# truemeat001/Simple-Raytracing-Render

Measured on AMD Instinct MI355X. Metric: Msamples/s (rays x bounces) + HBM GB/s vs roofline, Cornell+teapot 1024spp, higher is better.
Workload: dtype f32

## Files before the change

include/srr_capi.h:

```cpp
#ifndef SRR_CAPI_H
#define SRR_CAPI_H

#include <stddef.h>
#include <stdint.h>

#ifdef __cplusplus
extern "C" {
#endif

#define SRR_OK 0
#define SRR_EINVAL (-22)
#define SRR_ENOMEM (-12)
#define SRR_ENODEV (-19)
#define SRR_ENOTSUP (-95)
#define SRR_EIO (-5)

typedef struct srr_scene srr_scene;
typedef struct srr_renderer srr_renderer;

const char* srr_last_error(void);
const char* srr_version(void);

srr_scene* srr_scene_create(void);
void srr_scene_destroy(srr_scene* s);
int srr_scene_from_text(const char* text, srr_scene** out);
int srr_scene_text_handle(const srr_scene* s, int text_id);
int srr_scene_set_lcg(srr_scene* s, uint64_t state);
#define SRR_DIGEST_PARTS 21
int srr_scene_digest(const srr_scene* s, uint64_t* out, uint64_t* parts);
uint64_t srr_scene_get_lcg(const srr_scene* s);
double srr_scene_drand48(srr_scene* s);

int srr_constant_texture(srr_scene* s, float r, float g, float b);
int srr_image_texture(srr_scene* s, const unsigned char* rgb, int nx, int ny);
int srr_image_texture_file(srr_scene* s, const char* path);
int srr_image_texture_gen(srr_scene* s, int nx, int ny, uint32_t seed, int kind);
int srr_checker_texture(srr_scene* s, int even_tex, int odd_tex);
int srr_noise_texture(srr_scene* s, float scale);

int srr_lambertian(srr_scene* s, int albedo_tex);
int srr_orennayar(srr_scene* s, int albedo_tex, float sigma_deg);
int srr_beckmann(srr_scene* s, int albedo_tex, float roughx, float roughy);
int srr_metal(srr_scene* s, float r, float g, float b, float fuzz);
int srr_dielectric(srr_scene* s, float ref_idx);
int srr_diffuse_light(srr_scene* s, int emit_tex);
int srr_isotropic(srr_scene* s, int albedo_tex);

int srr_sphere(srr_scene* s, const float center[3], float radius, int mat);
int srr_moving_sphere(srr_scene* s, const float c0[3], const float c1[3], float t0, float t1, float radius,
                      int mat);
int srr_xy_rect(srr_scene* s, float x0, float x1, float y0, float y1, float k, int mat);
int srr_xz_rect(srr_scene* s, float x0, float x1, float z0, float z1, float k, int mat);
int srr_yz_rect(srr_scene* s, float y0, float y1, float z0, float z1, float k, int mat);
int srr_box(srr_scene* s, const float p0[3], const float p1[3], int mat);
int srr_triangle(srr_scene* s, const float p[9], int mat, const float* uv9, const float* n9);
int srr_flip_normals(srr_scene* s, int child);
int srr_translate(srr_scene* s, int child, const float offset[3]);
int srr_rotate_y(srr_scene* s, int child, float angle_deg);
int srr_rotate_x(srr_scene* s, int child, float angle_deg);
int srr_constant_medium(srr_scene* s, int boundary, float density, int tex);
int srr_hitable_list(srr_scene* s, const int* children, int n);
int srr_bvh_node(srr_scene* s, const int* children, int n, float time0, float time1);
int srr_teapot(srr_scene* s, float scale, int divs, int mat, int* first_handle);

int srr_model(srr_scene* s, const char* path, int flip_uvs, int flip_winding, int mat, const float scale[3],
              int* first_handle);
int srr_mesh_file_triangles(const char* path, int flip_uvs, int flip_winding, const float scale[3], float* pos9,
                            float* uv9, float* nrm9, int* flags_out);

int srr_camera(srr_scene* s, const float lookfrom[3], const float lookat[3], const float vup[3], float vfov,
               float aspect, float aperture, float focus_dist, float t0, float t1);
int srr_scene_set_world(srr_scene* s, int obj);
int srr_scene_set_lights(srr_scene* s, int list_obj);

typedef struct srr_params {
  int nx, ny;
  int spp;
  int max_depth;
  int tile;
  int shard_index;
  int shard_count;
  int batch_paths;
// ... 112 lines not shown
```

simple-raytracing-render_amd/csrc/capi.cpp:

```cpp
#include <hip/hip_runtime.h>

#include <algorithm>
#include <chrono>
#include <cstdint>
#include <cstdio>
#include <cstring>
#include <map>
#include <memory>
#include <mutex>
#include <string>
#include <vector>

#include "../../include/srr_capi.h"
#include "denoise.h"
#include "imageio.h"
#include "meshio.h"
#include "../../include/srr/merl.h"
#include "multi.h"
#include "renderer.h"

using namespace srr;

struct srr_scene {
  Scene s;
// ... 53 lines not shown
  std::string err;
  const int rc = flatten(s->s, f, err);
  if (rc < 0) return fail(rc, err);
  uint64_t h = 0xcbf29ce484222325ULL;
  int part = 0;
  auto mix = [](uint64_t& x, const void* p, size_t n) {
    const unsigned char* b = (const unsigned char*)p;
    for (size_t i = 0; i < n; ++i) x = (x ^ b[i]) * 0x100000001b3ULL;
  };
  auto blob = [&](const void* p, size_t n) {
    mix(h, &n, sizeof n);
    mix(h, p, n);
    if (const char* dd = getenv("SRR_DIGEST_DUMP")) {
      FILE* df = fopen((std::string(dd) + "." + std::to_string(part)).c_str(), "wb");
      if (df) { fwrite(p, 1, n, df); fclose(df); }
    }
    if (parts) {
      uint64_t x = 0xcbf29ce484222325ULL;
      mix(x, p, n);
      parts[part] = x;
    }
    ++part;
  };
  auto vec = [&blob](const auto& v) { blob(v.data(), v.size() * sizeof(v[0])); };
  vec(f.objs);
  blob(&f.n_world, sizeof f.n_world);
  vec(f.xforms);
  vec(f.spheres);
  vec(f.rects);
  vec(f.stris);
  vec(f.meshes);
  vec(f.nodes);
  vec(f.node4);
  vec(f.tri_pos);
  vec(f.tri_shade);
  vec(f.media);
  {
    std::vector<uint8_t> b;
    auto put = [&b](const void* p, size_t n) { b.insert(b.end(), (const uint8_t*)p, (const uint8_t*)p + n); };
    put(f.obvhs.data(), f.obvhs.size() * sizeof(DObvh));
    put(f.sgroups.data(), f.sgroups.size() * sizeof(DSGroup));
    put(f.sg_items.data(), f.sg_items.size() * sizeof(DSGItem));
    vec(b);
  }
  vec(f.obvh_children);
  vec(f.mats);
  vec(f.texs);
  vec(f.images);
  vec(f.perlin_ranvec);
  vec(f.perlin_perm);
  vec(f.lights);
  blob(&f.cam, sizeof f.cam);
  *out = h;
  return 0;
}

int srr_scene_set_lcg(srr_scene* s, uint64_t state) {
  if (!s) return fail(SRR_EINVAL, "null scene");
  s->s.lcg = state & 0xFFFFFFFFFFFFULL;
  return 0;
}
uint64_t srr_scene_get_lcg(const srr_scene* s) { return s ? s->s.lcg : 0; }
double srr_scene_drand48(srr_scene* s) { return s ? s->s.drand48() : 0.0; }

#define SCN(s) \
  if (!(s)) return fail(SRR_EINVAL, "null scene");
#define TEXOK(s, t) \
  if (!(s)->s.valid_tex(t)) return fail(SRR_EINVAL, "bad texture handle " + std::to_string(t));
#define MATOK(s, m) \
  if (!(s)->s.valid_mat(m)) return fail(SRR_EINVAL, "bad material handle " + std::to_string(m));
#define OBJOK(s, o) \
  if (!(s)->s.valid_obj(o)) return fail(SRR_EINVAL, "bad hitable handle " + std::to_string(o));

int srr_constant_texture(srr_scene* s, float r, float g, float b) {
  SCN(s);
  HTex t;
  t.kind = TEX_CONST;
  t.c[0] = r; t.c[1] = g; t.c[2] = b;
  return s->s.add_tex(std::move(t));
}
int srr_image_texture(srr_scene* s, const unsigned char* rgb, int nx, int ny) {
  SCN(s);
  if (!rgb || nx <= 0 || ny <= 0) return fail(SRR_EINVAL, "bad image");
  HTex t;
  t.kind = TEX_IMAGE;
  t.nx = nx;
  t.ny = ny;
  t.px.assign(rgb, rgb + (size_t)nx * ny * 3);
  return s->s.add_tex(std::move(t));
}
int srr_image_texture_file(srr_scene* s, const char* path) {
  SCN(s);
  if (!path) return fail(SRR_EINVAL, "null path");
  srr::Image im;
  std::string err;
  if (srr::load_image(path, 0, im, err) < 0) return fail(SRR_EIO, err);
  if (im.n < 3) return fail(SRR_EINVAL, std::string(path) + ": image_texture needs 3 or 4 channels");
  HTex t;
  t.kind = TEX_IMAGE;
  t.nx = im.w;
  t.ny = im.h;
  t.px.assign(im.px.begin(), im.px.begin() + (size_t)im.w * im.h * 3);
  return s->s.add_tex(std::move(t));
}
int srr_image_texture_gen(srr_scene* s, int nx, int ny, uint32_t seed, int kind) {
  SCN(s);
// ... 1088 lines not shown
```

simple-raytracing-render_amd/csrc/device_scene.h:

```cpp
#pragma once
#include <cstdint>

namespace srr {

enum ObjKind : int32_t {
  OBJ_SPHERE = 0,
  OBJ_MSPHERE = 1,
  OBJ_RECT = 2,
  OBJ_TRI = 3,
  OBJ_MESH = 4,
  OBJ_MEDIUM = 5,
  OBJ_OBVH = 6,
  OBJ_SGROUP = 7,
};

enum XformKind : int32_t { XF_FLIP = 0, XF_TRANSLATE = 1, XF_ROTY = 2, XF_ROTX = 3 };

struct DXform {
  int32_t kind;
  float a, b, c;
};


constexpr int32_t kXfFlipBit = 1 << 30;
constexpr int32_t kXfCountMask = 0xFFFF;

struct DObj {
  int32_t kind;
  int32_t xf_begin, xf_count;
  int32_t idx;
};

struct DSphere {
  float c0[3], c1[3];
  float t0, t1, r;
  int32_t mat;
};

struct DRect {
  int32_t kax, a0, a1, mat;
  float lo0, hi0, lo1, hi1, k;
  float pad[3];
};

struct TriShade {
  float n[9];
  float uv[6];
  int32_t mat;
};

constexpr int kNode4qWords = 16;

struct DMesh {
  int32_t node_off;
  int32_t tri_off;
  int32_t n_nodes, n_tris;
  int32_t node4_off;
  int32_t n_node4;
};

struct DObvh {
  int32_t node_off, n_nodes;
  int32_t child_off, n_children;
};

struct DObvhChild {
  int32_t obj_begin, obj_count;
};

constexpr int kSGroupMinRun = 8;

struct DSGroup {
  int32_t node_off, n_nodes;
  int32_t item_off, n_items;
};

struct DSGItem {
  DSphere s;
  int32_t pos;
  int32_t moving;
  int32_t obj;
  int32_t pad;
};

struct DMedium {
  int32_t bnd_begin, bnd_count;
  float density;
  int32_t phase_mat;
};

enum MatKind : int32_t {
  MAT_LAMBERTIAN = 0,
  MAT_ORENNAYAR = 1,
  MAT_BECKMANN = 2,
  MAT_METAL = 3,
  MAT_DIELECTRIC = 4,
// ... 40 lines not shown
```

simple-raytracing-render_amd/csrc/kernels.h:

```cpp
#pragma once
#include <hip/hip_runtime.h>

#include <cstdint>

#include "device_scene.h"

namespace srr {

struct SceneView {
  const DObj* objs;
  int n_world;
  int has_media;
  const DXform* xforms;
  const DSphere* spheres;
  const DRect* rects;
  const DStandaloneTri* stris;
  const DMesh* meshes;
  const float4* nodes;
  const float4* node4;
  int node4_lds;
  int node4_total;
  const float4* node4q;
  int node4_lds_q;
  int use_q;
  int quad_trace;
  int quad_max;
  int mesh_obj;
  const float4* tri_pos;
  const float4* tri_edge;
  const TriShade* tri_shade;
  const DMedium* media;
  const DObvh* obvhs;
  const DObvhChild* obvh_children;
  const DSGroup* sgroups;
  const DSGItem* sg_items;
  const DMat* mats;
  const DTex* texs;
  const uint8_t* images;
  const float* perlin_ranvec;
  const int32_t* perlin_perm;
  const DLight* lights;
  int n_lights;
  float light_weight;
  const DCamera* cam;
  const uint4* world_blob;
  int world_words;
  int world_off[10];
};

struct PathState {
  float4* ray_o;
  float4* ray_d;
  uint64_t* lcg;
  uint64_t* pcg;
  int32_t* depth;
  uint64_t* spec;
  int4* hit_w;
  float4* hit_p;
  float4* hit_n;
  float4* rec_a;
  float* sample;
  float* raw;
  uint8_t* rays;
};

struct BatchInfo {
  int32_t* active;
  int32_t* count;
  int act0;
  int slot0;
  const int32_t* pixels;
  const double* sobol;
  int p0;
  int n_paths;
  int s0, spp_batch;
  int s_base;
  int nx, ny;
  uint64_t base_seed;
};

struct UDiv31 {
  uint32_t m, p;
};
inline UDiv31 make_udiv31(uint32_t d) {
  uint32_t l = 0;
  while ((1ull << l) < d) ++l;
  const uint32_t p = 31 + l;
  return UDiv31{(uint32_t)(((1ull << p) + d - 1) / d), p};
}

struct PathWork {
  const int32_t* pixels;
  const double* sobol;
  int npix, spp_w;
  int s_base;
  int nx, ny;
  UDiv31 div_spp, div_nx;
  uint64_t base_seed;
  int64_t n_paths;
  int max_depth;
// ... 207 lines not shown
```

simple-raytracing-render_amd/csrc/kernels.hip:

```cpp
#include <hip/hip_runtime.h>

#include <cfloat>
#include <algorithm>
#include <cstdint>
#include <cstdlib>
#include <cstring>

#include "device_scene.h"
#include "devmath.h"
#include "kernels.h"
#include "../../include/srr/merl.h"

namespace srr {
namespace dev {

SRR_D V3 sphere_center(const DSphere& s, float tm, bool moving) {
  V3 c0 = v3(s.c0[0], s.c0[1], s.c0[2]);
  if (!moving) return c0;
  V3 c1 = v3(s.c1[0], s.c1[1], s.c1[2]);
  return c0 + ((tm - s.t0) / (s.t1 - s.t0)) * (c1 - c0);
}

SRR_D bool sphere_hit(const DSphere& s, bool moving, const Ray& r, float tmin, float tmax, float& t) {
  V3 oc = r.o - sphere_center(s, r.tm, moving);
// ... 598 lines not shown
    atomicAdd(cx.ctr + 1, (unsigned long long)ntri);
    if (overflow) atomicAdd(cx.ctr + 2, 1ull);
    const int steps = (int)(nbox / 4);
    atomicAdd(cx.ctr + 3 + min(steps, 63), 1ull);
    int wmax = steps;
    for (int o = 32; o > 0; o >>= 1) wmax = max(wmax, __shfl_xor(wmax, o));
    if ((int)__lane_id() == __ffsll((unsigned long long)__ballot(1)) - 1) atomicAdd(cx.ctr + 67 + min(wmax, 63), 1ull);
  }
  if (TIMING) {
    sp2 += __builtin_amdgcn_s_memtime() - ts;
    {
      int lm = (int)nbox;
      for (int o = 32; o > 0; o >>= 1) lm = max(lm, __shfl_xor(lm, o));
      const int src = __ffsll((unsigned long long)__ballot((int)nbox == lm)) - 1;
      cx.step_parts[0] += (uint64_t)__shfl((unsigned long long)sp0, src);
      cx.step_parts[1] += (uint64_t)__shfl((unsigned long long)sp1, src);
      cx.step_parts[2] += (uint64_t)__shfl((unsigned long long)sp2, src);
      cx.leaf_cycles += (uint64_t)__shfl((unsigned long long)slf, src);
      cx.leaf_passes += __shfl(spass, src);
    }
    int st = (int)(nbox / 4), sum = st, walk = st > 0;
    for (int o = 32; o > 0; o >>= 1) {
      st = max(st, __shfl_xor(st, o));
      sum += __shfl_xor(sum, o);
      walk += __shfl_xor(walk, o);
    }
    cx.mesh_steps += st;
    cx.mesh_lane_steps += sum;
    cx.mesh_walkers += walk;
    cx.mesh_cycles += __builtin_amdgcn_s_memtime() - tm_enter;
  }
  if (cx.ovf && cx.gst) {
    const uint64_t dm = __ballot(deep && !suspended);
    if (dm && (int)__lane_id() == __ffsll((unsigned long long)dm) - 1) atomicAdd(cx.ovf + (kCtrDeepTraversals - kCtrStackOverflows), (unsigned long long)__popcll(dm));
  }
#ifdef SRR_SLOW_RAYS
  cx.last_steps += (int)(nbox / 4) | (overflow ? 1 << 30 : 0) | (deep ? 1 << 29 : 0);
#endif
  if (SUSP && suspended) return false;
  if (overflow) {
    if (cx.ovf) atomicAdd(cx.ovf, 1ull);
    return mesh_hit<false>(S, m, r, tmin, tmax, is_medium, out, cx.ctr);
  }
  out.t = best_t;
  out.tri = best_i;
  return found;
}

constexpr int TR_QUAD = 32;
constexpr int TR_Q = 64;
constexpr int TR_BIG = 128;
constexpr int tr_stride(int tr) { return (tr & TR_BIG) ? 1024 : kTraceBlock; }
constexpr int TR_SUSP = 256;

template <int CTRL>
SRR_D int quad_dpp(int x) { return __builtin_amdgcn_update_dpp(x, x, CTRL, 0xF, 0xF, false); }
template <int CTRL>
SRR_D float quad_dpp(float x) { return __int_as_float(quad_dpp<CTRL>(__float_as_int(x))); }
constexpr int kQuadXor1 = 0xB1, kQuadXor2 = 0x4E;
template <int K>
constexpr int kQuadBcast = K * 0x55;

SRR_D void quad_best(bool& f, float& t, int& i) {
#define SRR_QSTEP(CTRL)                                                      \
  {                                                                          \
    const bool of = quad_dpp<CTRL>((int)f) != 0;                             \
    const float ot = quad_dpp<CTRL>(t);                                      \
    const int oi = quad_dpp<CTRL>(i);                                        \
    if (of && (!f || wins(ot, oi, t, i))) { f = true; t = ot; i = oi; }       \
  }
  SRR_QSTEP(kQuadXor1) SRR_QSTEP(kQuadXor2)
#undef SRR_QSTEP
}

template <bool PRUNE, int STRIDE = kTraceBlock>
SRR_D bool mesh_hit4_quad(const SceneView& S, const DMesh& m, const Ray& r, float tmin, float tmax, bool is_medium,
                          MeshHit& out, const TraceCtx& cx) {
  if (const uint64_t nanm = __ballot(!(tmax == tmax))) {
    bool f = false;
    float bt = 0;
    int bi = -1;
    mesh_scan_nan(S, m, r, is_medium, nanm, f, bt, bi);
    if (!(tmax == tmax)) {
#ifdef SRR_SLOW_RAYS
      cx.last_steps |= 1 << 28;
#endif
      out.t = bt;
      out.tri = bi;
      return f;
    }
  }
  const V3 inv = v3(1.0f / r.d.x, 1.0f / r.d.y, 1.0f / r.d.z);
  const bool want = slab(S.nodes[2 * m.node_off], S.nodes[2 * m.node_off + 1], r.o, inv, tmin, tmax);
  if (__ballot(1) != ~0ull) {
    if (!want) return false;
    return mesh_hit4<PRUNE, false, false, STRIDE>(S, m, r, tmin, tmax, is_medium, out, cx);
  }
  const int lane = __lane_id(), q = lane >> 2, c = lane & 3;
  const float len = length(r.d);
  const V3 dir = r.d / len;
  const float to_param = kPruneSlack / len;
  const int gslot = cx.slot - c;
  bool found_me = false, redo_me = false;
  float t_me = 0;
  int i_me = -1;
  uint64_t W = __ballot(want);
// ... 409 lines not shown
  float lo = -FLT_MAX;
#pragma unroll 1
  for (int pass = 0; pass < 2; ++pass) {
    float th;
    if (!list_hit<TR>(S, md.bnd_begin, md.bnd_count, r, lo, FLT_MAX, th, cx)) return false;
    tb[pass] = th;
    lo = (float)((double)th + 0.0001);
  }
  float t1 = tb[0], t2 = tb[1];
  if (t1 < tmin) t1 = tmin;
  if (t2 > tmax) t2 = tmax;
  if (t1 >= t2) return false;
  if (t1 < 0) t1 = 0;
  float len = length(r.d);
  float inside = (t2 - t1) * len;
  float hit_distance = -(1 / md.density) * gm64::log(drand(rng));
  if (hit_distance < inside) {
    t = t1 + hit_distance / len;
    return true;
  }
  return false;
}

struct WorldHit {
  int obj;
  int prim;
  float t;
};

template <bool MEDIA, int TR>
SRR_D void world_objs(const SceneView& S, const Ray& r, Rng& rng, const TraceCtx& cx, int k0, int k1, WorldHit& w,
                      float& closest) {
  const float tmin = 0.001f;
  for (int k = k0; k < k1; ++k) {
    const DObj ob = uni(wload<TR>(S.objs, k));
    Ray lr = chain_in<TR, true>(S, ob, r);
    ObjHit h;
    bool hit;
    if (MEDIA && ob.kind == OBJ_MEDIUM) {
      hit = medium_hit<TR>(S, uni(wload<TR>(S.media, ob.idx)), lr, tmin, closest, rng, h.t, cx);
      h.prim = -1;
    } else {
      hit = basic_hit<TR, true>(S, ob, lr, tmin, closest, false, h, cx);
    }
    if (hit) {
      closest = h.t;
      w.obj = k;
      w.prim = h.prim;
      w.t = h.t;
    }
  }
}

template <bool MEDIA, int TR>
SRR_D WorldHit world_hit(const SceneView& S, const Ray& r, Rng& rng, const TraceCtx& cx) {
  WorldHit w{-1, -1, 0};
  float closest = FLT_MAX;
  const float tmin = 0.001f;
  constexpr bool SUSP = (TR & TR_SUSP) != 0;
  const bool skip = MEDIA || S.mesh_obj < 0;
  int k_res = -1;
  if constexpr (SUSP) {
    if (skip && cx.resume) {
      const float4 v = *walk_save(cx, 2);
      k_res = __float_as_int(v.x);
      closest = v.y;
      w.obj = __float_as_int(v.z);
      w.prim = __float_as_int(v.w);
      w.t = closest;
    }
  }
  for (int k = 0; k < S.n_world; ++k) {
    const DObj ob = uni(wload<TR>(S.objs, k));
    if constexpr (SUSP) {
      if (skip && (cx.susp || k < k_res)) continue;
      cx.obj_k = k;
    }
    Ray lr = chain_in<TR, true>(S, ob, r);
    ObjHit h;
    bool hit;
    if (MEDIA && ob.kind == OBJ_MEDIUM) {
      hit = medium_hit<TR>(S, uni(wload<TR>(S.media, ob.idx)), lr, tmin, closest, rng, h.t, cx);
      h.prim = -1;
    } else {
      hit = basic_hit<TR, true>(S, ob, lr, tmin, closest, false, h, cx);
    }
    if (SUSP && skip && cx.susp) {
      *walk_save(cx, 2) = make_float4(__int_as_float(k), closest, __int_as_float(w.obj), __int_as_float(w.prim));
      continue;
    }
    if (hit) {
      closest = h.t;
      w.obj = k;
      w.prim = h.prim;
      w.t = h.t;
    }
  }
  return w;
}

struct HitRec {
  V3 p, n;
  float u, v;
  int mat;
};

template <int KAX>
SRR_D void rect_rec(const DRect& q, const Ray& r, HitRec& h) {
  constexpr int A0 = KAX == 0 ? 1 : 0, A1 = KAX == 2 ? 1 : 2;
  const float tt = (q.k - r.o[KAX]) / r.d[KAX];
  const float x = r.o[A0] + tt * r.d[A0];
  const float y = r.o[A1] + tt * r.d[A1];
  h.u = (x - q.lo0) / (q.hi0 - q.lo0);
  h.v = (y - q.lo1) / (q.hi1 - q.lo1);
  h.n = v3(0.f);
  h.n.set(KAX, 1.f);
}

SRR_D void sphere_uv(V3 p, float& u, float& v) {
  float phi = ratan2(p.z, p.x);
  float theta = rasin(p.y);
  u = 1 - (phi + kPi) / (2 * kPi);
  v = (theta + kPi / 2) / kPi;
}

// ... 1436 lines not shown
      e[12] = __int_as_float(wh.prim);
      e[13] = wh.t;
      e[14] = __int_as_float(slot);
      e[15] = __int_as_float((int)(t_w0 & 0x7fffffff));
    }
  }
}
#endif

constexpr int kTpWords = 8, kTfWords = kCtrBeckAttemptsMax - kCtrTicksBeck + 1, kTzWords = 2, kTptWords = 3;
constexpr int kTpPhases = kCtrTicksFold - kCtrTicksRefill + 1;
template <int Q>
constexpr int tp_at() {
  constexpr int at = Q >= kCtrTicksRefill && Q <= kCtrTicksFold ? Q - kCtrTicksRefill
                     : Q == kCtrTicksRecord ? kTpPhases : Q == kCtrTicksMixture ? kTpPhases + 1
                     : Q == kCtrMixtureRounds ? kTpPhases + 2 : -1;
  static_assert(at >= 0 && at < kTpWords, "not a word of tp");
  return at;
}
template <int Q>
constexpr int tf_at() {
  static_assert(Q >= kCtrTicksBeck && Q <= kCtrBeckAttemptsMax, "not a word of tf");
  return Q - kCtrTicksBeck;
}
template <int Q>
constexpr int tz_at() {
  static_assert(Q >= kCtrTicksCamOnly && Q < kCtrTicksCamOnly + kTzWords, "not a word of tz");
  return Q - kCtrTicksCamOnly;
}
template <int Q>
constexpr int tpt_at() {
  static_assert(Q >= kCtrTicksPretrace && Q < kCtrTicksPretrace + kTptWords, "not a word of tpt");
  return Q - kCtrTicksPretrace;
}
constexpr int kThtWords = kCtrTailLanes - kCtrTicksHead + 1;
constexpr int kHeadLiveMin = 32;

template <bool MEDIA, bool ALLFAM, int MINB, bool TIMED = false, bool WL = true, bool QUAD = false, bool CQ = false,
          int BS = kPathsBlock, bool SP = false>
#ifdef SRR_NUM_VGPR
#define SRR_PATHS_VGPR_ATTR __attribute__((amdgpu_num_vgpr(SRR_NUM_VGPR)))
#else
#define SRR_PATHS_VGPR_ATTR
#endif
__global__ void __launch_bounds__(BS, MINB) SRR_PATHS_VGPR_ATTR k_paths(PathsArgs A) {
  static_assert(BS == kPathsBlock || BS == 1024, "block size");
  (void)A;
  uint64_t tp[kTpWords] = {0, 0, 0, 0, 0, 0, 0, 0};
  uint64_t tf[kTfWords] = {0, 0, 0, 0, 0, 0, 0, 0, 0, 0, 0, 0, 0, 0, 0, 0, 0, 0, 0, 0};
  uint64_t tz[kTzWords] = {0, 0};
  uint64_t it = 0;
  uint64_t tpt[kTptWords] = {0, 0, 0};
  constexpr int TR = TR_BVH4_PRUNE | (WL ? TR_WL : 0) | (QUAD ? TR_QUAD : 0) | (CQ ? TR_Q : 0) | (BS == 1024 ? TR_BIG : 0) |
                     ((SP && !QUAD && !CQ) ? TR_SUSP : 0);
  __shared__ uint4 s_world[WL ? kWorldLdsBytes / 16 : 1];
  const auto view = [&]() {
    SceneView S = paths_args()->S;
    if constexpr (WL) {
      const char* b = (const char*)s_world;
      S.objs = (const DObj*)(b + S.world_off[0]);
      S.xforms = (const DXform*)(b + S.world_off[1]);
      S.spheres = (const DSphere*)(b + S.world_off[2]);
      S.rects = (const DRect*)(b + S.world_off[3]);
      S.stris = (const DStandaloneTri*)(b + S.world_off[4]);
      S.meshes = (const DMesh*)(b + S.world_off[5]);
      S.media = (const DMedium*)(b + S.world_off[6]);
      S.mats = (const DMat*)(b + S.world_off[7]);
      S.texs = (const DTex*)(b + S.world_off[8]);
      S.lights = (const DLight*)(b + S.world_off[9]);
    }
    return S;
  };
  const auto work = []() { return PathWork(paths_args()->W); };
  __shared__ int s_node[kStack * BS];
  __shared__ float s_t[kStack * BS];
  constexpr bool RING = !QUAD;
  constexpr bool PT = RING && !MEDIA && !ALLFAM && (BS == 1024 || TIMED);
  constexpr int kRingWords = ring_words(PT);
  constexpr int kNodesLds = paths_lds_nodes(BS, WL, RING, PT);
  static_assert(paths_lds_fits(BS, WL, RING, PT), "k_paths LDS");
  __shared__ float4 s_n4[kNodesLds * 8];
  __shared__ float s_ring[RING ? kRingWords * BS : 1];
  static_assert(sizeof(s_world) + sizeof(s_node) + sizeof(s_t) + sizeof(s_n4) + sizeof(s_ring) ==
                    (size_t)paths_lds_bytes(BS, WL, RING, PT), "k_paths LDS as kernels.h counts it");
  const auto lds_nodes = [](const SceneView& S) { return min(S.node4_total, (CQ ? 2 : 1) * kNodesLds); };
  const lds_ptr<float> ringw = to_lds(s_ring + (RING ? (threadIdx.x & ~63u) : 0));
  uint32_t ring_base = 0;
  const uint32_t n_paths = (uint32_t)paths_args()->W.n_paths;
  const uint64_t t_start = paths_args()->W.wave_times ? __builtin_amdgcn_s_memrealtime() : 0;
  {
    const SceneView S0 = paths_args()->S;
    if constexpr (WL)
      for (int i = threadIdx.x; i < S0.world_words; i += blockDim.x) s_world[i] = S0.world_blob[i];
    const int n_lds_nodes = lds_nodes(S0);
    if (CQ)
      for (int i = threadIdx.x; i < n_lds_nodes * 4; i += blockDim.x) s_n4[i] = S0.node4q[i];
    else
      for (int i = threadIdx.x; i < n_lds_nodes * 8; i += blockDim.x) s_n4[i] = S0.node4[i];
  }
  __syncthreads();
  const int slot = blockIdx.x * blockDim.x + threadIdx.x;
  const auto rec_at = [&](const PathWork& W, int k) -> float4* {
    int s = slot;
    asm volatile("" : "+v"(s));
    return W.rec + ((size_t)k * W.lanes + s);
  };
  int g = -1;
// ... 134 lines not shown
          if (lane_id() == 0) b = (uint32_t)atomicAdd(W.cursor, (unsigned long long)kPoolChunk);
          nb = __builtin_amdgcn_readfirstlane(b);
        }
        idx = rank < avail ? pool + rank : nb + (rank - avail);
        pool = nb + (cnt - avail);
        pool_end = nb + (uint32_t)kPoolChunk;
      }
      if (!RING && need && idx < n_paths) {
        g = (int)idx;
        path_camera_ray(S, W, idx, r, rng);
        depth = 0;
      }
    }
    if (!nxt_armed && pool_end < n_paths) {
      nxt_lane0 = pool_arm(nxt_lane0);
      nxt_armed = true;
    }
    if (__ballot(g >= 0) == 0) break;
    if (TIMED) tf[tf_at<kCtrLanesInPath>()] += __popcll(__ballot(g >= 0));
    if (TIMED) {
      __builtin_amdgcn_s_waitcnt(0);
      const uint64_t t = __builtin_amdgcn_s_memtime();
      tp[tp_at<kCtrTicksRefill>()] += t - tq;
      tq = t;
      ++it;
    }
    }
    const bool head_now = PT && !tail;
    const bool act = g >= 0;
    const Ray tr = r;
    if (act) {
      const SceneView S = view();
      const PathWork W = work();
      TraceCtx cx{nullptr, to_lds(s_node + threadIdx.x), to_lds(s_t + threadIdx.x)};
      cx.lds_nodes = (const __attribute__((address_space(3))) f32x4*)to_lds(s_n4);
      cx.lds_count = lds_nodes(S);
      cx.st_cap = min(W.stack_cap, kStack);
      cx.ovf = W.counters + kCtrStackOverflows;
      cx.gst = W.gstack;
      cx.gst_cap = W.gstack ? W.gstack_cap : 0;
      cx.gst_stride = W.lanes;
      cx.slot = slot;
      if constexpr ((TR & TR_SUSP) != 0) {
        cx.walk_thr = vreg(head_now ? 0 : (int)((__popcll(__ballot(true)) * (uint32_t)paths_args()->W.walk_q) >> 6));
        cx.resume = walking;
        cx.susp = vreg(0);
      }
#ifdef SRR_SLOW_RAYS
      const uint64_t t_w0 = __builtin_amdgcn_s_memrealtime();
      cx.last_steps = 0;
      const Ray r_in = tr;
#endif
      const WorldHit wh =
          world_hit<MEDIA, TIMED ? (TR_BVH4_TIMED | (WL ? TR_WL : 0) | (SP ? TR_SUSP : 0)) : TR>(S, tr, rng, cx);
      w = wh;
      if constexpr ((TR & TR_SUSP) != 0) {
        walking = cx.susp;
        if (walking) {
          w.obj = -1;
          n_events += kSuspended;
        }
      }
#ifdef SRR_SLOW_RAYS
      slow_ray_record(W, g, depth, r_in, t_w0, cx.last_steps, wh, slot);
#endif
      if (TIMED) {
        const uint64_t t = __builtin_amdgcn_s_memtime();
        if (head_now && passes == 0) {
          tpt[tpt_at<kCtrTicksPretrace>()] += t - tq;
          ++tpt[tpt_at<kCtrPretracePasses>()];
        } else {
          if (__ballot(depth != 0) == 0) {
            tz[tz_at<kCtrTicksCamOnly>()] += t - tq;
            ++tz[tz_at<kCtrItsCamOnly>()];
          }
          tp[tp_at<kCtrTicksWorld>()] += t - tq - cx.mesh_cycles;
          tp[tp_at<kCtrTicksMesh>()] += cx.mesh_cycles;
          tf[tf_at<kCtrMeshSteps>()] += cx.mesh_steps;
          tf[tf_at<kCtrMeshLaneSteps>()] += cx.mesh_lane_steps;
          tf[tf_at<kCtrMeshWalkers>()] += cx.mesh_walkers;
          tf[tf_at<kCtrLeafTicks>()] += cx.leaf_cycles;
          tf[tf_at<kCtrLeafPasses>()] += cx.leaf_passes;
          tf[tf_at<kCtrStepFetch>()] += cx.step_parts[0];
          tf[tf_at<kCtrStepSlab>()] += cx.step_parts[1];
          tf[tf_at<kCtrStepOrder>()] += cx.step_parts[2];
        }
        tq = t;
      }
    }
    if (nxt_armed && !nxt_ready) {
      nxt_base = __builtin_amdgcn_readfirstlane(nxt_lane0);
      nxt_ready = true;
    }
    {
    const bool sh = g >= 0 && !(PT && walking);
    if (PT && TIMED) ++tpt[tpt_at<kCtrShadeRounds>()];
    bool done = sh && !walking;
    V3 C = v3(0.f);
    bool diff = false, pend = false;
    int natt = 0;
    uint64_t fam_dt[3] = {0, 0, 0};
    DiffSetup ds{};
    V3 d_atten = v3(0.f), d_n = v3(0.f), d_dir = v3(0.f);
    float d_pdf = 0;
    int d_tries = 0;
    bool d_dead = false;
    if (sh) {
// ... 1254 lines not shown
```

simple-raytracing-render_amd/csrc/renderer.cpp:

```cpp
#include "renderer.h"

#include "multi.h"

#include <algorithm>
#include <chrono>
#include <cstdlib>
#include <cstring>
#include <memory>
#include <thread>
#include <cstdio>

namespace srr {

constexpr int kVisitWords = 3 + 2 * 64;

#define RCHK(x)                                                        \
  do {                                                                 \
    hipError_t e_ = (x);                                               \
    if (e_ != hipSuccess) {                                            \
      err = std::string(#x) + ": " + hipGetErrorString(e_);            \
      return SRR_EIO;                                                  \
    }                                                                  \
  } while (0)

// ... 19 lines not shown
  r->device = device;
  if (const char* e = getenv("SRR_LANES")) r->n_lanes = std::max(1, std::min(kMaxLanes, atoi(e)));
  RCHK(hipSetDevice(device));
  std::vector<void*>& K = r->scene_bufs;
  DObj* objs; DXform* xf; DSphere* sph; DRect* rct; DStandaloneTri* st; DMesh* me; float* nodes; float* n4;
  float* tp; TriShade* ts; DMedium* md; DMat* mt; DTex* tx; uint8_t* im; float* pr; int32_t* pp; DLight* li;
  DCamera* cm;
  DObvh* ob;
  DObvhChild* oc;
  DSGroup* sg;
  DSGItem* sgi;
  std::vector<DCamera> cam{F.cam};
  RCHK(upload(&objs, F.objs, K));
  RCHK(upload(&xf, F.xforms, K));
  RCHK(upload(&sph, F.spheres, K));
  RCHK(upload(&rct, F.rects, K));
  RCHK(upload(&st, F.stris, K));
  RCHK(upload(&me, F.meshes, K));
  RCHK(upload(&nodes, F.nodes, K));
  RCHK(upload(&n4, F.node4, K));
  float* n4q;
  RCHK(upload(&n4q, F.node4q, K));
  RCHK(upload(&tp, F.tri_pos, K));
  float* tedge;
  {
    const size_t nt = F.tri_pos.size() / 16;
    std::vector<float> pr(32 * nt, 0.f);
    for (size_t i = 0; i < nt; ++i)
      for (int j = 0; j < 2; ++j) {
        const float* q = &F.tri_pos[16 * std::min(i + j, nt - 1)];
        float* o = &pr[32 * i + 9 * j];
        for (int c = 0; c < 3; ++c) {
          o[c] = q[c];
          o[3 + c] = q[4 + c] - q[c];
          o[6 + c] = q[8 + c] - q[c];
        }
      }
    RCHK(upload(&tedge, pr, K));
  }
  RCHK(upload(&ts, F.tri_shade, K));
  RCHK(upload(&md, F.media, K));
  RCHK(upload(&ob, F.obvhs, K));
  RCHK(upload(&oc, F.obvh_children, K));
  RCHK(upload(&sg, F.sgroups, K));
  RCHK(upload(&sgi, F.sg_items, K));
  RCHK(upload(&mt, F.mats, K));
  RCHK(upload(&tx, F.texs, K));
  RCHK(upload(&im, F.images, K));
  RCHK(upload(&pr, F.perlin_ranvec, K));
  RCHK(upload(&pp, F.perlin_perm, K));
  RCHK(upload(&li, F.lights, K));
  RCHK(upload(&cm, cam, K));
  std::vector<uint8_t> blob;
  int off[10];
  auto put = [&](int k, const void* data, size_t bytes) {
    off[k] = (int)blob.size();
    blob.insert(blob.end(), (const uint8_t*)data, (const uint8_t*)data + bytes);
    blob.resize((blob.size() + 15) & ~(size_t)15, 0);
  };
  put(0, F.objs.data(), F.objs.size() * sizeof(DObj));
  put(1, F.xforms.data(), F.xforms.size() * sizeof(DXform));
  put(2, F.spheres.data(), F.spheres.size() * sizeof(DSphere));
  put(3, F.rects.data(), F.rects.size() * sizeof(DRect));
  put(4, F.stris.data(), F.stris.size() * sizeof(DStandaloneTri));
  put(5, F.meshes.data(), F.meshes.size() * sizeof(DMesh));
  put(6, F.media.data(), F.media.size() * sizeof(DMedium));
  put(7, F.mats.data(), F.mats.size() * sizeof(DMat));
  put(8, F.texs.data(), F.texs.size() * sizeof(DTex));
  put(9, F.lights.data(), F.lights.size() * sizeof(DLight));
  uint8_t* wb;
  RCHK(upload(&wb, blob, K));
  SceneView& V = r->view;
  V.world_blob = (const uint4*)wb;
  V.world_words = (int)(blob.size() / 16);
  for (int k = 0; k < 10; ++k) V.world_off[k] = off[k];
  V.objs = objs;
  V.n_world = F.n_world;
  V.has_media = F.media.empty() ? 0 : 1;
  V.xforms = xf;
  V.spheres = sph;
  V.rects = rct;
  V.stris = st;
  V.meshes = me;
  V.nodes = (const float4*)nodes;
  V.node4 = (const float4*)n4;
  V.node4_lds = (int)std::min<size_t>(kPathsLdsNodes, F.node4.size() / 32);
  V.node4_total = (int)(F.node4.size() / 32);
  V.node4q = F.node4q_ok && !F.node4q.empty() ? (const float4*)n4q : nullptr;
  V.node4_lds_q = (int)std::min<size_t>(2 * kPathsLdsNodes, F.node4q.size() / kNode4qWords);
  {
    const char* e = getenv("SRR_CBVH");
    V.use_q = V.node4q && e && atoi(e) != 0;
  }
  {
    const char* e = getenv("SRR_QUAD");
    V.quad_trace = e ? (atoi(e) != 0) : false;
    const char* q = getenv("SRR_QUAD_MAX");
    V.quad_max = q ? atoi(q) : 32;
  }
  {
    int n_mesh = 0;
    V.mesh_obj = -1;
    for (int k = 0; k < F.n_world; ++k)
      if (F.objs[k].kind == OBJ_MESH) {
        ++n_mesh;
        V.mesh_obj = k;
      }
    if (n_mesh != 1) V.mesh_obj = -1;
  }
  V.tri_pos = (const float4*)tp;
  V.tri_edge = (const float4*)tedge;
  V.tri_shade = ts;
  V.media = md;
  V.obvhs = ob;
  V.obvh_children = oc;
  V.sgroups = sg;
  V.sg_items = sgi;
  V.mats = mt;
  V.texs = tx;
  V.images = im;
  V.perlin_ranvec = pr;
  V.perlin_perm = pp;
  V.lights = li;
  V.n_lights = (int)F.lights.size();
  V.light_weight = V.n_lights > 0 ? (float)(1.0 / V.n_lights) : 0.f;
  V.cam = cm;
  r->has_meshes = !F.meshes.empty() || !F.obvhs.empty();
  r->diffuse_only = true;
// ... 1185 lines not shown
```

simple-raytracing-render_amd/csrc/scene.cpp:

```cpp
#include "scene.h"

#include <algorithm>
#include <array>
#include <cfloat>
#include <cmath>
#include <cstdio>
#include <cstdlib>
#include <cstring>
#include <fstream>
#include <functional>
#include <iterator>
#include <map>
#include <sstream>

namespace srr {

static const double kPi = 3.14159265358979323846;
static const uint64_t kPostPerlinSeed = 24561125610955ULL;

#include "../../include/srr/teapot_data.inc"

Scene::Scene() : lcg(kPostPerlinSeed) {}

double Scene::drand48() {
// ... 1317 lines not shown
    g.item_off = (int)F.sg_items.size();
    g.n_items = (int)items.size();
    std::vector<float> nodes;
    std::function<void(int, int)> build = [&](int lo, int hi) {
      double mn[3] = {INFINITY, INFINITY, INFINITY}, mx[3] = {-INFINITY, -INFINITY, -INFINITY};
      double cmn[3] = {INFINITY, INFINITY, INFINITY}, cmx[3] = {-INFINITY, -INFINITY, -INFINITY};
      for (int k = lo; k < hi; ++k)
        for (int a = 0; a < 3; ++a) {
          mn[a] = std::min(mn[a], items[k].mn[a]);
          mx[a] = std::max(mx[a], items[k].mx[a]);
          cmn[a] = std::min(cmn[a], items[k].c[a]);
          cmx[a] = std::max(cmx[a], items[k].c[a]);
        }
      const size_t me = nodes.size() / 8;
      nodes.resize(nodes.size() + 8);
      for (int a = 0; a < 3; ++a) {
        float fl = (float)mn[a], fh = (float)mx[a];
        if ((double)fl > mn[a]) fl = std::nextafter(fl, -INFINITY);
        if ((double)fh < mx[a]) fh = std::nextafter(fh, INFINITY);
        nodes[8 * me + a] = fl;
        nodes[8 * me + 4 + a] = fh;
      }
      int32_t leaf = -1;
      if (hi - lo <= 2) {
        leaf = ((int)F.sg_items.size() << 1) | (hi - lo - 1);
        for (int k = lo; k < hi; ++k) F.sg_items.push_back(items[k].it);
      } else {
        int ax = 0;
        for (int a = 1; a < 3; ++a)
          if (cmx[a] - cmn[a] > cmx[ax] - cmn[ax]) ax = a;
        const int mid = (lo + hi) / 2;
        std::nth_element(items.begin() + lo, items.begin() + mid, items.begin() + hi,
                         [ax](const It& x, const It& y) { return x.c[ax] < y.c[ax]; });
        build(lo, mid);
        build(mid, hi);
      }
      const int32_t skip = g.node_off + (int32_t)(nodes.size() / 8);
      std::memcpy(&nodes[8 * me + 3], &skip, 4);
      std::memcpy(&nodes[8 * me + 7], &leaf, 4);
    };
    build(0, (int)items.size());
    g.n_nodes = (int)(nodes.size() / 8);
    F.nodes.insert(F.nodes.end(), nodes.begin(), nodes.end());
    F.sgroups.push_back(g);
    DObj d{};
    d.kind = OBJ_SGROUP;
    d.idx = (int)F.sgroups.size() - 1;
    out.push_back(d);
    i = j;
  }
  return out;
}

int flatten(const Scene& S, Flat& F, std::string& err) {
  F = Flat();
  if (S.world < 0 || S.lights < 0 || !S.has_camera) {
    err = "scene needs world, lights and a camera";
    return -22;
  }
  if (S.obj[S.lights].kind != H_LIST) {
    err = "lights must be a hitable_list (Raytracing_n.cpp:75 casts it)";
    return -22;
  }
  for (const HMat& m : S.mat) {
    DMat d{};
    d.kind = m.kind;
    d.tex = m.tex;
    std::memcpy(d.p, m.p, 16);
    F.mats.push_back(d);
  }
  for (const HTex& t : S.tex) {
    DTex d{};
    d.kind = t.kind;
    std::memcpy(d.c, t.c, 12);
    d.nx = t.nx;
    d.ny = t.ny;
    d.even = t.even;
    d.odd = t.odd;
    if (t.kind == TEX_IMAGE) {
      d.off = (int64_t)F.images.size();
      F.images.insert(F.images.end(), t.px.begin(), t.px.end());
    }
    F.texs.push_back(d);
  }
  Flattener fl{S, F, err};
  if (!fl.walk(S.world, {}, fl.world, false)) return -95;
  std::vector<DObj> grouped_objs;
  const std::vector<DObj> world = group_sphere_runs(S, F, fl.world, grouped_objs);
  F.n_world = (int)world.size();
  F.objs = world;
  for (DObj d : fl.bound) F.objs.push_back(d);
  for (DMedium& m : F.media) m.bnd_begin += F.n_world;
  const int inner_base = (int)F.objs.size();
  for (DObj d : fl.inner) F.objs.push_back(d);
  for (DObvhChild& c : F.obvh_children) c.obj_begin += inner_base;
  const int grouped_base = (int)F.objs.size();
  for (DObj d : grouped_objs) F.objs.push_back(d);
  for (DSGItem& it : F.sg_items) it.obj += grouped_base;
  for (int k : S.obj[S.lights].kids) {
    if (S.obj[k].kind == H_LIST) {
      err = "nested hitable_list inside the light list is not supported";
      return -95;
    }
    F.lights.push_back(fl.light(k));
  }
  compact_materials(F);
  perlin_tables(F.perlin_ranvec, F.perlin_perm);
  const HCamera& c = S.cam;
  std::memcpy(F.cam.origin, c.origin, 12);
  std::memcpy(F.cam.llc, c.llc, 12);
  std::memcpy(F.cam.horizontal, c.horizontal, 12);
  std::memcpy(F.cam.vertical, c.vertical, 12);
  std::memcpy(F.cam.u, c.u, 12);
  std::memcpy(F.cam.v, c.v, 12);
  F.cam.time0 = c.time0;
  F.cam.time1 = c.time1;
  F.cam.lens_radius = c.lens_radius;
  return 0;
}

namespace {
struct Tok {
  std::vector<std::string> t;
  int line;
  float f(size_t i) const { return std::strtof(t.at(i).c_str(), nullptr); }
  long long i(size_t k) const { return std::strtoll(t.at(k).c_str(), nullptr, 10); }
  unsigned long long u(size_t k) const { return std::strtoull(t.at(k).c_str(), nullptr, 10); }
  void v3(size_t k, float* o) const { o[0] = f(k); o[1] = f(k + 1); o[2] = f(k + 2); }
};
}

int scene_from_text(const std::string& text, Scene& S, std::string& err) {
  std::istringstream is(text);
  std::string line;
  int ln = 0;
  bool header = false;
  std::map<long long, int> T, M, O;
  std::map<long long, std::pair<int, int>> G;
  auto need = [&](std::map<long long, int>& mp, long long id, const char* what) -> int {
    if (id == -1 && std::string(what) == "mat") return -1;
    auto it = mp.find(id);
    if (it == mp.end()) throw std::runtime_error(std::string("undefined ") + what + " " + std::to_string(id));
    return it->second;
  };
  try {
    while (std::getline(is, line)) {
      ++ln;
      size_t h = line.find('#');
      if (h != std::string::npos) line.resize(h);
      Tok c;
      c.line = ln;
      std::istringstream ls(line);
      std::string w;
      while (ls >> w) c.t.push_back(w);
      if (c.t.empty()) continue;
      const std::string& k = c.t[0];
      if (!header) {
        if (k != "srr_scene" || c.i(1) != 1) throw std::runtime_error("not an srr_scene v1 description");
        header = true;
// ... 110 lines not shown
```

simple-raytracing-render_amd/csrc/scene.h:

```cpp
#pragma once
#include <cstdint>
#include <string>
#include <vector>

#include "device_scene.h"

namespace srr {

enum HKind : int32_t {
  H_SPHERE, H_MSPHERE, H_XY, H_XZ, H_YZ, H_BOX, H_TRI, H_FLIP, H_TRANSLATE, H_ROTY, H_ROTX, H_MEDIUM, H_LIST, H_BVH
};

struct Box3 {
  float mn[3], mx[3];
};

struct HTex {
  TexKind kind;
  float c[3] = {0, 0, 0};
  int nx = 0, ny = 0;
  std::vector<uint8_t> px;
  int even = -1, odd = -1;
};

// ... 57 lines not shown

  int add_tex(HTex t);
  int add_mat(HMat m);
  int add_obj(HObj o);
  int material(MatKind k, int tex, const float* prm);
  int sphere(const float c[3], float r, int m);
  int moving_sphere(const float c0[3], const float c1[3], float t0, float t1, float r, int m);
  int rect(HKind k, float a0, float a1, float b0, float b1, float kk, int m);
  int box(const float p0[3], const float p1[3], int m);
  int triangle(const float p[9], int m, const float* uv9, const float* n9);
  int wrap(HKind k, int child, const float* f);
  int rotate(HKind k, int child, float angle);
  int medium(int boundary, float density, int tex);
  int list(const int* kids, int n);
  int bvh(const int* kids, int n, float t0, float t1);
  int teapot(float scale, int divs, int m, int* first);
  void camera(const float lf[3], const float la[3], const float vup[3], float vfov, float aspect, float aperture,
              float focus, float t0, float t1);

  bool bbox(int h, float t0, float t1, Box3& b) const;
  bool valid_obj(int h) const { return h >= 0 && h < (int)obj.size(); }
  bool valid_mat(int m) const { return m == -1 || (m >= 0 && m < (int)mat.size()); }
  bool valid_tex(int t) const { return t >= 0 && t < (int)tex.size(); }
};

int scene_from_text(const std::string& text, Scene& s, std::string& err);

struct Flat {
  std::vector<DObj> objs;
  int n_world = 0;
  std::vector<DXform> xforms;
  std::vector<DSphere> spheres;
  std::vector<DRect> rects;
  std::vector<DStandaloneTri> stris;
  std::vector<DMesh> meshes;
  std::vector<float> nodes;
  std::vector<float> node4;
  std::vector<float> node4q;
  bool node4q_ok = true;
  std::vector<float> tri_pos;
  std::vector<TriShade> tri_shade;
  std::vector<DMedium> media;
  std::vector<DObvh> obvhs;
  std::vector<DObvhChild> obvh_children;
  std::vector<DSGroup> sgroups;
  std::vector<DSGItem> sg_items;
  std::vector<DMat> mats;
  std::vector<DTex> texs;
  std::vector<uint8_t> images;
  std::vector<float> perlin_ranvec;
  std::vector<int32_t> perlin_perm;
  std::vector<DLight> lights;
  DCamera cam{};
};

int flatten(const Scene& s, Flat& f, std::string& err);

void teapot_triangles(float scale, int divs, std::vector<float>& p9);

uint64_t path_seed(uint32_t x, uint32_t y, uint32_t s, uint64_t base);

void sobol2(unsigned n, double* out);

std::vector<uint8_t> gen_image(int w, int h, uint32_t seed, int kind);

}
```

simple-raytracing-render_amd/srr/capi.py:

```python
from __future__ import annotations

import ctypes
import os

import numpy as np

PKG = os.path.dirname(os.path.dirname(os.path.abspath(__file__)))
LIB_PATH = os.environ.get("SRR_LIB") or os.path.join(PKG, "libsrr.so")
_LIB = None

FLAG_SORT_MATERIALS = 1
FLAG_KEEP_PATHS = 2
FLAG_COUNT_VISITS = 4
FLAG_WAVEFRONT = 8
FLAG_CONTINUE = 16
FLAG_SUMS = 32
AOV_ALBEDO = 1
AOV_NORMAL = 2
AOV_DEPTH = 4
DENOISE_DEMODULATE = 1


class SrrError(RuntimeError):
    pass
# ... 284 lines not shown
    def render_device_async(self, params: Params, d_mean_ptr: int) -> int:
        t = ctypes.c_int64()
        _check(lib().srr_render_device_async(self.h, ctypes.byref(params), ctypes.c_void_p(d_mean_ptr),
                                             ctypes.byref(t)))
        return t.value

    def wait(self, ticket: int) -> dict:
        st = Stats()
        _check(lib().srr_render_wait(self.h, ctypes.c_int64(ticket), ctypes.byref(st)))
        return st.as_dict()


def adaptive_converged(n, s1, s2, rel_tol, abs_eps) -> bool:
    return bool(lib().srr_adaptive_converged(int(n), float(s1), float(s2), float(rel_tol), float(abs_eps)))


def denoise(color, albedo, normal, depth, params: DenoiseParams = None, device: int = 0) -> np.ndarray:
    color = np.ascontiguousarray(color, np.float32)
    if color.ndim != 3 or color.shape[2] != 3:
        raise SrrError("denoise needs color[ny, nx, 3]")
    ny, nx = color.shape[:2]
    albedo = np.ascontiguousarray(albedo, np.float32)
    normal = np.ascontiguousarray(normal, np.float32)
    depth = np.ascontiguousarray(depth, np.float32)
    if albedo.size != color.size or normal.size != color.size or depth.size * 3 != color.size:
        raise SrrError("denoise: albedo and normal need ny*nx*3 floats, depth ny*nx")
    dp = params if params is not None else DenoiseParams.defaults()
    out = np.zeros_like(color)
    _check(lib().srr_denoise_host(device, nx, ny, ctypes.byref(dp), _ptr(color), _ptr(albedo), _ptr(normal),
                                  _ptr(depth), _ptr(out)))
    return out


def tonemap(mean: np.ndarray) -> np.ndarray:
    mean = np.ascontiguousarray(mean, np.float32)
    out = np.zeros(mean.shape, np.uint8)
    _check(lib().srr_tonemap(_ptr(mean), mean.size // 3, _ptr(out)))
    return out


def scene_digest(text: str) -> str:
    L = lib()
    L.srr_scene_digest.argtypes = [ctypes.c_void_p, ctypes.POINTER(ctypes.c_uint64), ctypes.c_void_p]
    h = ctypes.c_void_p()
    _check(L.srr_scene_from_text(text.encode(), ctypes.byref(h)))
    d = ctypes.c_uint64()
    try:
        _check(L.srr_scene_digest(h, ctypes.byref(d), None))
    finally:
        L.srr_scene_destroy(h)
    return f"{d.value:016x}"


def write_ppm(path: str, nx: int, ny: int, img8: np.ndarray) -> None:
    img8 = np.ascontiguousarray(img8, np.uint8)
    _check(lib().srr_write_ppm(path.encode(), nx, ny, _ptr(img8)))


def image_load(path: str, req_comp: int = 0) -> tuple[np.ndarray, int]:
    x, y, n = ctypes.c_int(), ctypes.c_int(), ctypes.c_int()
    p = ctypes.POINTER(ctypes.c_ubyte)()
    ch = _check(lib().srr_image_load(path.encode(), req_comp, ctypes.byref(x), ctypes.byref(y), ctypes.byref(n),
                                     ctypes.byref(p)))
    try:
        px = np.ctypeslib.as_array(p, shape=(y.value, x.value, ch)).copy()
    finally:
        lib().srr_image_free(p)
    return px, n.value


def write_png(path: str, nx: int, ny: int, img8: np.ndarray) -> None:
    img8 = np.ascontiguousarray(img8, np.uint8)
    if img8.size != nx * ny * 3:
        raise SrrError("write_png needs nx*ny*3 bytes")
    _check(lib().srr_write_png(path.encode(), nx, ny, _ptr(img8)))


def mesh_file_triangles(path: str, flip_uvs: bool = False, flip_winding: bool = False, scale=(1.0, 1.0, 1.0)):
    sc = np.ascontiguousarray(scale, np.float32)
    fl = ctypes.c_int(0)
    n = _check(lib().srr_mesh_file_triangles(path.encode(), int(flip_uvs), int(flip_winding), _ptr(sc), None, None,
                                             None, ctypes.byref(fl)))
    pos, uv, nrm = (np.zeros((n, 3, 3), np.float32) for _ in range(3))
    _check(lib().srr_mesh_file_triangles(path.encode(), int(flip_uvs), int(flip_winding), _ptr(sc), _ptr(pos),
                                         _ptr(uv), _ptr(nrm), None))
    return pos, uv, nrm, bool(fl.value & 1), bool(fl.value & 2)
```

Baseline: 9910.

## Batch consecutive plain world rects into packed runs tested without per-object dispatch

At flatten time, consecutive top-level world objects that are untransformed axis-aligned rects are grouped into segments. Each segment gets a compact 6-word record per rect, stored in the world blob. The trace kernel walks segments instead of individual objects and tests each run in groups of four, using one vector load per group and branchless hit updates. This is meant to cut per-object DObj loads and kind dispatch for the Cornell box walls. It adds a switch on the axis per rect and extra padding, and routes every world_hit instantiation through the new path. A C API and Python helper are added to inspect the segment tables.

```diff
diff --git a/include/srr_capi.h b/include/srr_capi.h
--- a/include/srr_capi.h
+++ b/include/srr_capi.h
@@ -28,6 +28,8 @@
 int srr_scene_set_lcg(srr_scene* s, uint64_t state);
 #define SRR_DIGEST_PARTS 21
 int srr_scene_digest(const srr_scene* s, uint64_t* out, uint64_t* parts);
+int srr_scene_world_segments(const srr_scene* s, int32_t* counts, int32_t* segs, int cap_segs, int32_t* run_rects,
+                             int cap_run_rects, int32_t* objs, int cap_objs, int32_t* rects, int cap_rects);
 uint64_t srr_scene_get_lcg(const srr_scene* s);
 double srr_scene_drand48(srr_scene* s);
 
diff --git a/simple-raytracing-render_amd/csrc/capi.cpp b/simple-raytracing-render_amd/csrc/capi.cpp
--- a/simple-raytracing-render_amd/csrc/capi.cpp
+++ b/simple-raytracing-render_amd/csrc/capi.cpp
@@ -129,6 +129,30 @@
   vec(f.lights);
   blob(&f.cam, sizeof f.cam);
   *out = h;
+  return 0;
+}
+
+int srr_scene_world_segments(const srr_scene* s, int32_t* counts, int32_t* segs, int cap_segs, int32_t* run_rects,
+                             int cap_run_rects, int32_t* objs, int cap_objs, int32_t* rects, int cap_rects) {
+  if (!s || !counts) return fail(SRR_EINVAL, "null argument");
+  Flat f;
+  std::string err;
+  const int rc = flatten(s->s, f, err);
+  if (rc < 0) return fail(rc, err);
+  static_assert(sizeof(DSeg) == 16 && sizeof(DObj) == 16 && sizeof(DRect) == 48,
+"table rows as srr_capi.h describes them");
+  counts[0] = f.n_world;
+  counts[1] = (int32_t)f.segs.size();
+  counts[2] = (int32_t)(f.run_rects.size() / kRunRectWords);
+  counts[3] = (int32_t)f.objs.size();
+  counts[4] = (int32_t)f.rects.size();
+  const auto copy = [](int32_t* dst, int cap, const void* src, size_t bytes) {
+    if (dst && cap > 0 && bytes > 0) std::memcpy(dst, src, std::min(bytes, (size_t)cap * 4));
+  };
+  copy(segs, cap_segs, f.segs.data(), f.segs.size() * sizeof(DSeg));
+  copy(run_rects, cap_run_rects, f.run_rects.data(), f.run_rects.size() * 4);
+  copy(objs, cap_objs, f.objs.data(), f.objs.size() * sizeof(DObj));
+  copy(rects, cap_rects, f.rects.data(), f.rects.size() * sizeof(DRect));
   return 0;
 }
 
diff --git a/simple-raytracing-render_amd/csrc/device_scene.h b/simple-raytracing-render_amd/csrc/device_scene.h
--- a/simple-raytracing-render_amd/csrc/device_scene.h
+++ b/simple-raytracing-render_amd/csrc/device_scene.h
@@ -42,6 +42,12 @@
   float lo0, hi0, lo1, hi1, k;
   float pad[3];
 };
+
+struct DSeg {
+  int32_t first, count, rect0, pad;
+};
+constexpr int kRunRectWords = 6;
+constexpr int kRunGroup = 4;
 
 struct TriShade {
   float n[9];
diff --git a/simple-raytracing-render_amd/csrc/kernels.h b/simple-raytracing-render_amd/csrc/kernels.h
--- a/simple-raytracing-render_amd/csrc/kernels.h
+++ b/simple-raytracing-render_amd/csrc/kernels.h
@@ -45,7 +45,10 @@
   const DCamera* cam;
   const uint4* world_blob;
   int world_words;
-  int world_off[10];
+  int world_off[12];
+  const DSeg* segs;
+  int n_segs;
+  const int32_t* run_rects;
 };
 
 struct PathState {
diff --git a/simple-raytracing-render_amd/csrc/kernels.hip b/simple-raytracing-render_amd/csrc/kernels.hip
--- a/simple-raytracing-render_amd/csrc/kernels.hip
+++ b/simple-raytracing-render_amd/csrc/kernels.hip
@@ -674,6 +674,7 @@
 constexpr int TR_BIG = 128;
 constexpr int tr_stride(int tr) { return (tr & TR_BIG) ? 1024 : kTraceBlock; }
 constexpr int TR_SUSP = 256;
+constexpr int TR_RUNS = 512;
 
 template <int CTRL>
 SRR_D int quad_dpp(int x) { return __builtin_amdgcn_update_dpp(x, x, CTRL, 0xF, 0xF, false); }
@@ -1189,6 +1190,45 @@
   }
 }
 
+template <int KAX>
+SRR_D void run_rect(const int32_t* q, const Ray& r, float tmin, int id, float& closest, int& obj) {
+  constexpr int A0 = KAX == 0 ? 1 : 0, A1 = KAX == 2 ? 1 : 2;
+  const float k = __int_as_float(q[1]), lo0 = __int_as_float(q[2]), hi0 = __int_as_float(q[3]);
+  const float lo1 = __int_as_float(q[4]), hi1 = __int_as_float(q[5]);
+  const float tt = (k - r.o[KAX]) / r.d[KAX];
+  const float x = r.o[A0] + tt * r.d[A0];
+  const float y = r.o[A1] + tt * r.d[A1];
+  const bool out_t = (tt < tmin) | (tt > closest);
+  const bool out_xy = (x < lo0) | (x > hi0) | (y < lo1) | (y > hi1);
+  const bool hit = !out_t & !out_xy;
+  closest = hit ? tt : closest;
+  obj = hit ? id : obj;
+}
+
+struct RunGroup {
+  int32_t w[kRunGroup * kRunRectWords];
+};
+SRR_D void rect_run_fold(const SceneView& S, const DSeg& sg, const Ray& r, float tmin, WorldHit& w, float& closest) {
+  int obj = w.obj;
+  for (int i0 = 0; i0 < sg.count; i0 += kRunGroup) {
+    const RunGroup g = cload((const RunGroup*)(S.run_rects + kRunRectWords * (sg.rect0 + i0)), 0);
+#pragma unroll
+    for (int j = 0; j < kRunGroup; ++j) {
+      if (i0 + j < sg.count) {
+        const int32_t* q = g.w + kRunRectWords * j;
+        const int id = sg.first + i0 + j;
+        switch (q[0]) {
+          case 0: run_rect<0>(q, r, tmin, id, closest, obj); break;
+          case 1: run_rect<1>(q, r, tmin, id, closest, obj); break;
+          default: run_rect<2>(q, r, tmin, id, closest, obj); break;
+        }
+      }
+    }
+  }
+  w.t = obj != w.obj ? closest : w.t;
+  w.obj = obj;
+}
+
 template <bool MEDIA, int TR>
 SRR_D WorldHit world_hit(const SceneView& S, const Ray& r, Rng& rng, const TraceCtx& cx) {
   WorldHit w{-1, -1, 0};
@@ -1207,7 +1247,18 @@
       w.t = closest;
     }
   }
-  for (int k = 0; k < S.n_world; ++k) {
+  constexpr bool RUNS = (TR & TR_RUNS) != 0;
+  const int n_steps = RUNS ? S.n_segs : S.n_world;
+  for (int step = 0; step < n_steps; ++step) {
+    int k = step;
+    if constexpr (RUNS) {
+      const DSeg sg = cload(S.segs, step);
+      if (sg.count != 0) {
+        if (!(SUSP && skip && (cx.susp || sg.first < k_res))) rect_run_fold(S, sg, r, tmin, w, closest);
+        continue;
+      }
+      k = sg.first;
+    }
     const DObj ob = uni(wload<TR>(S.objs, k));
     if constexpr (SUSP) {
       if (skip && (cx.susp || k < k_res)) continue;
@@ -2750,7 +2801,7 @@
   uint64_t it = 0;
   uint64_t tpt[kTptWords] = {0, 0, 0};
   constexpr int TR = TR_BVH4_PRUNE | (WL ? TR_WL : 0) | (QUAD ? TR_QUAD : 0) | (CQ ? TR_Q : 0) | (BS == 1024 ? TR_BIG : 0) |
-                     ((SP && !QUAD && !CQ) ? TR_SUSP : 0);
+                     ((SP && !QUAD && !CQ) ? TR_SUSP : 0) | TR_RUNS;
   __shared__ uint4 s_world[WL ? kWorldLdsBytes / 16 : 1];
   const auto view = [&]() {
     SceneView S = paths_args()->S;
@@ -2991,7 +3042,7 @@
       const Ray r_in = tr;
 #endif
       const WorldHit wh =
-          world_hit<MEDIA, TIMED ? (TR_BVH4_TIMED | (WL ? TR_WL : 0) | (SP ? TR_SUSP : 0)) : TR>(S, tr, rng, cx);
+          world_hit<MEDIA, TIMED ? (TR_BVH4_TIMED | (WL ? TR_WL : 0) | (SP ? TR_SUSP : 0) | TR_RUNS) : TR>(S, tr, rng, cx);
       w = wh;
       if constexpr ((TR & TR_SUSP) != 0) {
         walking = cx.susp;
diff --git a/simple-raytracing-render_amd/csrc/renderer.cpp b/simple-raytracing-render_amd/csrc/renderer.cpp
--- a/simple-raytracing-render_amd/csrc/renderer.cpp
+++ b/simple-raytracing-render_amd/csrc/renderer.cpp
@@ -95,7 +95,7 @@
   RCHK(upload(&li, F.lights, K));
   RCHK(upload(&cm, cam, K));
   std::vector<uint8_t> blob;
-  int off[10];
+  int off[12];
   auto put = [&](int k, const void* data, size_t bytes) {
     off[k] = (int)blob.size();
     blob.insert(blob.end(), (const uint8_t*)data, (const uint8_t*)data + bytes);
@@ -111,12 +111,17 @@
   put(7, F.mats.data(), F.mats.size() * sizeof(DMat));
   put(8, F.texs.data(), F.texs.size() * sizeof(DTex));
   put(9, F.lights.data(), F.lights.size() * sizeof(DLight));
+  put(10, F.segs.data(), F.segs.size() * sizeof(DSeg));
+  put(11, F.run_rects.data(), F.run_rects.size() * sizeof(int32_t));
   uint8_t* wb;
   RCHK(upload(&wb, blob, K));
   SceneView& V = r->view;
   V.world_blob = (const uint4*)wb;
   V.world_words = (int)(blob.size() / 16);
-  for (int k = 0; k < 10; ++k) V.world_off[k] = off[k];
+  for (int k = 0; k < 12; ++k) V.world_off[k] = off[k];
+  V.segs = (const DSeg*)(wb + off[10]);
+  V.n_segs = (int)F.segs.size();
+  V.run_rects = (const int32_t*)(wb + off[11]);
   V.objs = objs;
   V.n_world = F.n_world;
   V.has_media = F.media.empty() ? 0 : 1;
diff --git a/simple-raytracing-render_amd/csrc/scene.cpp b/simple-raytracing-render_amd/csrc/scene.cpp
--- a/simple-raytracing-render_amd/csrc/scene.cpp
+++ b/simple-raytracing-render_amd/csrc/scene.cpp
@@ -1393,6 +1393,32 @@
   return out;
 }
 
+void world_segments(Flat& F) {
+  F.segs.clear();
+  F.run_rects.clear();
+  const auto plain_rect = [&F](int k) {
+    return F.objs[k].kind == OBJ_RECT && (F.objs[k].xf_count & kXfCountMask) == 0;
+  };
+  for (int k = 0; k < F.n_world;) {
+    int e = k;
+    while (e < F.n_world && plain_rect(e)) ++e;
+    if (e - k < 2) {
+      F.segs.push_back(DSeg{k, 0, 0, 0});
+      ++k;
+      continue;
+    }
+    F.segs.push_back(DSeg{k, e - k, (int32_t)(F.run_rects.size() / kRunRectWords), 0});
+    for (; k < e; ++k) {
+      const DRect& q = F.rects[F.objs[k].idx];
+      const float f[kRunRectWords - 1] = {q.k, q.lo0, q.hi0, q.lo1, q.hi1};
+      int32_t w[kRunRectWords] = {q.kax, 0, 0, 0, 0, 0};
+      std::memcpy(w + 1, f, sizeof f);
+      F.run_rects.insert(F.run_rects.end(), w, w + kRunRectWords);
+    }
+  }
+  if (!F.run_rects.empty()) F.run_rects.resize(F.run_rects.size() + (kRunGroup - 1) * kRunRectWords, 0);
+}
+
 int flatten(const Scene& S, Flat& F, std::string& err) {
   F = Flat();
   if (S.world < 0 || S.lights < 0 || !S.has_camera) {
@@ -1446,6 +1472,7 @@
     F.lights.push_back(fl.light(k));
   }
   compact_materials(F);
+  world_segments(F);
   perlin_tables(F.perlin_ranvec, F.perlin_perm);
   const HCamera& c = S.cam;
   std::memcpy(F.cam.origin, c.origin, 12);
diff --git a/simple-raytracing-render_amd/csrc/scene.h b/simple-raytracing-render_amd/csrc/scene.h
--- a/simple-raytracing-render_amd/csrc/scene.h
+++ b/simple-raytracing-render_amd/csrc/scene.h
@@ -133,9 +133,13 @@
   std::vector<int32_t> perlin_perm;
   std::vector<DLight> lights;
   DCamera cam{};
+  std::vector<DSeg> segs;
+  std::vector<int32_t> run_rects;
 };
 
 int flatten(const Scene& s, Flat& f, std::string& err);
+
+void world_segments(Flat& f);
 
 void teapot_triangles(float scale, int divs, std::vector<float>& p9);
 
diff --git a/simple-raytracing-render_amd/srr/capi.py b/simple-raytracing-render_amd/srr/capi.py
--- a/simple-raytracing-render_amd/srr/capi.py
+++ b/simple-raytracing-render_amd/srr/capi.py
@@ -360,6 +360,27 @@
     return f"{d.value:016x}"
 
 
+def world_segments(text: str) -> dict:
+    L = lib()
+    i32p = ctypes.POINTER(ctypes.c_int32)
+    L.srr_scene_world_segments.argtypes = [ctypes.c_void_p, i32p, i32p, ctypes.c_int, i32p, ctypes.c_int, i32p,
+                                           ctypes.c_int, i32p, ctypes.c_int]
+    h = ctypes.c_void_p()
+    _check(L.srr_scene_from_text(text.encode(), ctypes.byref(h)))
+    try:
+        counts = (ctypes.c_int32 * 5)()
+        _check(L.srr_scene_world_segments(h, counts, None, 0, None, 0, None, 0, None, 0))
+        n_world, n_segs, n_rows, n_objs, n_rects = (int(c) for c in counts)
+        tabs = {"segs": np.zeros((n_segs, 4), np.int32), "run_rects": np.zeros((n_rows, 6), np.int32),
+                "objs": np.zeros((n_objs, 4), np.int32), "rects": np.zeros((n_rects, 12), np.int32)}
+        p = {k: (v.ctypes.data_as(i32p) if v.size else None, int(v.size)) for k, v in tabs.items()}
+        _check(L.srr_scene_world_segments(h, counts, *p["segs"], *p["run_rects"], *p["objs"], *p["rects"]))
+    finally:
+        L.srr_scene_destroy(h)
+    tabs["n_world"] = n_world
+    return tabs
+
+
 def write_ppm(path: str, nx: int, ny: int, img8: np.ndarray) -> None:
     img8 = np.ascontiguousarray(img8, np.uint8)
     _check(lib().srr_write_ppm(path.encode(), nx, ny, _ptr(img8)))
```

Result: no change. 9956, median of 6 (+0.5%).
